# eric-downes/tianshou_marl

Measured on AMD Instinct MI355X. Metric: env-steps/sec (n_env x n_agent) incl. PPO update, simple_spread N=3, higher is better.
Workload: dtype f32; 1 GPU; simple_spread_v3 N=3 shared PPO, num_envs=1024 per GPU, obs 18, A=5, T=25, MLP 64-64; minibatch=4096, repeat=1, dispatch=per_agent, parallelism=env-shard x1

## Files before the change

tianshou_marl_amd/csrc/mlp_tile.h:

```cpp
#pragma once
#include "common.h"

namespace {

typedef float f4 __attribute__((ext_vector_type(4)));

constexpr int R = 16;
constexpr int NT = 256;
constexpr int kMaxJ = 4;

struct Dims {
    int D, A;
    int Kp1;
    int nJ;
    int ld1;
};

__host__ __device__ constexpr Dims dims_const(int D, int A) {
    Dims d{};
    d.D = D; d.A = A; d.Kp1 = (D + 3) / 4 * 4; d.nJ = (D + 15) / 16; d.ld1 = 16 * ((D + 15) / 16) + 2;
    return d;
}

template <int H>
struct Lay {
    static constexpr int ldh = H + 2;
    static constexpr int ld2 = 2 * H + 2;
    static constexpr int ldo = 18;
    int W1, W2a, W2c, W3a, W3c, B1, B2, B3a, B3c, X, H1, H2, OUT, D3, D2, D1, total;
    __host__ __device__ Lay(const Dims &d, bool bwd) {
        int o = 0;
        W1 = o; o += 2 * H * d.ld1;
        W2a = o; o += H * ldh;
        W2c = o; o += H * ldh;
        W3a = o; o += 16 * ldh;
        W3c = o; o += H;
        B1 = o; o += 2 * H;
        B2 = o; o += 2 * H;
        B3a = o; o += 16;
        B3c = o; o += 2;
        o = (o + 3) & ~3;
        X = o; o += R * d.ld1;
        H1 = o; o += R * ld2;
        H2 = o; o += R * ld2;
        OUT = o; o += R * ldo;
        D3 = o; o += bwd ? R * ldo : 0;
        D2 = o; o += bwd ? R * ld2 : 0;
        D1 = o; o += bwd ? R * ld2 : 0;
        total = o;
    }
};

__device__ __forceinline__ f4 mfma(float a, float b, f4 c) {
    return __builtin_amdgcn_mfma_f32_16x16x4f32(a, b, c, 0, 0, 0);
}

template <int N>
__device__ __forceinline__ float fmaf_chain_ahead(const float *h, const float *w) {
    constexpr int Q = 8;
    static_assert(N % (2 * Q) == 0, "pairs of whole groups");
    float h0[Q], w0[Q], h1[Q], w1[Q], s = 0.f;
    int off = 0;
    auto pin = [&]() { asm volatile("" : "+v"(s), "+v"(off)); };
#pragma unroll
    for (int p = 0; p < Q; ++p) { h0[p] = h[p]; w0[p] = w[p]; }
#pragma unroll
    for (int j0 = 0; j0 < N; j0 += 2 * Q) {
        pin();
#pragma unroll
        for (int p = 0; p < Q; ++p) { h1[p] = h[off + j0 + Q + p]; w1[p] = w[off + j0 + Q + p]; }
#pragma unroll
        for (int p = 0; p < Q; ++p) s = fmaf(h0[p], w0[p], s);
        pin();
        if (j0 + 2 * Q < N) {
#pragma unroll
            for (int p = 0; p < Q; ++p) { h0[p] = h[off + j0 + 2 * Q + p]; w0[p] = w[off + j0 + 2 * Q + p]; }
        }
#pragma unroll
        for (int p = 0; p < Q; ++p) s = fmaf(h1[p], w1[p], s);
    }
    return s;
}

template <int H>
struct POff {
    int aW1, ab1, aW2, ab2, aW3, ab3, cW1, cb1, cW2, cb2, cW3, cb3, total;
    __host__ __device__ POff(int D, int A) {
        int o = 0;
        aW1 = o; o += H * D; ab1 = o; o += H; aW2 = o; o += H * H; ab2 = o; o += H; aW3 = o; o += A * H; ab3 = o; o += A;
        cW1 = o; o += H * D; cb1 = o; o += H; cW2 = o; o += H * H; cb2 = o; o += H; cW3 = o; o += H; cb3 = o; o += 1;
        total = o;
    }
};

template <int H>
__device__ void stage_weights(float *lds, const Lay<H> &ly, const Dims &d, const float *__restrict__ P, int tid_in = -1) {
    const POff<H> po(d.D, d.A);
    const int tid = tid_in < 0 ? (int)threadIdx.x : tid_in;
    constexpr int U = 12;
    for (int e0 = tid; e0 < 2 * H * d.ld1; e0 += U * NT) {
        float v[U];
#pragma unroll
        for (int u = 0; u < U; ++u) {
            const int e = e0 + u * NT;
            const int row = e / d.ld1, c = e - row * d.ld1;
            v[u] = 0.f;
            if (e < 2 * H * d.ld1 && c < d.D) v[u] = row < H ? P[po.aW1 + row * d.D + c] : P[po.cW1 + (row - H) * d.D + c];
        }
#pragma unroll
        for (int u = 0; u < U; ++u)
            if (e0 + u * NT < 2 * H * d.ld1) lds[ly.W1 + e0 + u * NT] = v[u];
    }
    for (int e0 = tid; e0 < H * ly.ldh; e0 += U * NT) {
        float va[U], vc[U];
#pragma unroll
        for (int u = 0; u < U; ++u) {
            const int e = e0 + u * NT;
            const int row = e / ly.ldh, c = e - row * ly.ldh;
            const bool on = e < H * ly.ldh && c < H;
            va[u] = on ? P[po.aW2 + row * H + c] : 0.f;
            vc[u] = on ? P[po.cW2 + row * H + c] : 0.f;
        }
#pragma unroll
        for (int u = 0; u < U; ++u) {
            const int e = e0 + u * NT;
            if (e < H * ly.ldh) { lds[ly.W2a + e] = va[u]; lds[ly.W2c + e] = vc[u]; }
        }
    }
    {
        constexpr int N3 = (16 * Lay<H>::ldh + NT - 1) / NT;
        float v3[N3], vv[5];
#pragma unroll
        for (int u = 0; u < N3; ++u) {
            const int e = tid + u * NT, row = e / ly.ldh, c = e - row * ly.ldh;
            v3[u] = (e < 16 * ly.ldh && row < d.A && c < H) ? P[po.aW3 + row * H + c] : 0.f;
        }
        const int e5 = tid < H ? tid : 0;
        vv[0] = P[po.cW3 + e5]; vv[1] = P[po.ab1 + e5]; vv[2] = P[po.cb1 + e5]; vv[3] = P[po.ab2 + e5]; vv[4] = P[po.cb2 + e5];
#pragma unroll
        for (int u = 0; u < N3; ++u) {
            const int e = tid + u * NT;
            if (e < 16 * ly.ldh) lds[ly.W3a + e] = v3[u];
        }
        if (tid < H) {
            lds[ly.W3c + tid] = vv[0]; lds[ly.B1 + tid] = vv[1]; lds[ly.B1 + H + tid] = vv[2]; lds[ly.B2 + tid] = vv[3];
            lds[ly.B2 + H + tid] = vv[4];
        }
    }
    if (tid < 16) lds[ly.B3a + tid] = tid < d.A ? P[po.ab3 + tid] : 0.f;
    if (tid == 0) lds[ly.B3c] = P[po.cb3];
}

constexpr int kStageChunk = 4 * 256;
__host__ __device__ inline int image_f4_padded(int x_floats) {
    return ((x_floats / 4) + kStageChunk - 1) / kStageChunk * kStageChunk;
}

template <int H>
__device__ __forceinline__ void stage_image(float *lds, const Lay<H> &ly, const float *__restrict__ img) {
    const int n4p = image_f4_padded(ly.X);
    const int wave_base = (threadIdx.x >> 6) * 64;
    for (int e = 0; e < n4p; e += NT) {
        __builtin_amdgcn_global_load_lds(
            (const __attribute__((address_space(1))) void *)(img + (size_t)(e + threadIdx.x) * 4),
            (__attribute__((address_space(3))) void *)(lds + (size_t)(e + wave_base) * 4), 16, 0, 0);
    }
}

template <int H>
__device__ __forceinline__ void tile_forward(float *lds, const Lay<H> &ly, const Dims &d) {
    const int lane = threadIdx.x & 63, w = threadIdx.x >> 6;
    const int r16 = lane & 15, kq = lane >> 4;
    {
        f4 acc_a = {0.f, 0.f, 0.f, 0.f}, acc_c = {0.f, 0.f, 0.f, 0.f};
        const float *xa = lds + ly.X + r16 * d.ld1 + kq;
        const float *wa = lds + ly.W1 + (16 * w + r16) * d.ld1 + kq;
        const float *wc = lds + ly.W1 + (H + 16 * w + r16) * d.ld1 + kq;
        for (int k0 = 0; k0 < d.Kp1; k0 += 4) {
            const float a = xa[k0];
            acc_a = mfma(a, wa[k0], acc_a);
            acc_c = mfma(a, wc[k0], acc_c);
        }
        const int col = 16 * w + r16;
        const float ba = lds[ly.B1 + col], bc = lds[ly.B1 + H + col];
#pragma unroll
        for (int r = 0; r < 4; ++r) {
            const int row = kq * 4 + r;
            lds[ly.H1 + row * ly.ld2 + col] = fmaxf(acc_a[r] + ba, 0.f);
            lds[ly.H1 + row * ly.ld2 + H + col] = fmaxf(acc_c[r] + bc, 0.f);
        }
    }
    __syncthreads();
    {
        f4 acc_a = {0.f, 0.f, 0.f, 0.f}, acc_c = {0.f, 0.f, 0.f, 0.f};
        const float *ha = lds + ly.H1 + r16 * ly.ld2 + kq;
        const float *hc = ha + H;
        const float *wa = lds + ly.W2a + (16 * w + r16) * ly.ldh + kq;
        const float *wc = lds + ly.W2c + (16 * w + r16) * ly.ldh + kq;
#pragma unroll
        for (int k0 = 0; k0 < H; k0 += 4) {
            acc_a = mfma(ha[k0], wa[k0], acc_a);
            acc_c = mfma(hc[k0], wc[k0], acc_c);
        }
        const int col = 16 * w + r16;
        const float ba = lds[ly.B2 + col], bc = lds[ly.B2 + H + col];
#pragma unroll
        for (int r = 0; r < 4; ++r) {
            const int row = kq * 4 + r;
            lds[ly.H2 + row * ly.ld2 + col] = fmaxf(acc_a[r] + ba, 0.f);
            lds[ly.H2 + row * ly.ld2 + H + col] = fmaxf(acc_c[r] + bc, 0.f);
        }
    }
    __syncthreads();
    if (w == 0) {
        f4 acc = {0.f, 0.f, 0.f, 0.f};
        const float *ha = lds + ly.H2 + r16 * ly.ld2 + kq;
        const float *wa = lds + ly.W3a + r16 * ly.ldh + kq;
#pragma unroll
        for (int k0 = 0; k0 < H; k0 += 4) acc = mfma(ha[k0], wa[k0], acc);
        const float b = lds[ly.B3a + r16];
#pragma unroll
        for (int r = 0; r < 4; ++r) lds[ly.OUT + (kq * 4 + r) * ly.ldo + r16] = acc[r] + b;
    } else if (w == 1 && lane < R) {
        const float *hc = lds + ly.H2 + lane * ly.ld2 + H;
        float s = 0.f;
        for (int j = 0; j < H; ++j) s = fmaf(hc[j], lds[ly.W3c + j], s);
        lds[ly.OUT + lane * ly.ldo + 16] = s + lds[ly.B3c];
    }
    __syncthreads();
}

template <int H>
__device__ __forceinline__ void tile_forward_split(float *lds, const Lay<H> &ly, const Dims &d) {
    const int lane = threadIdx.x & 63, w8 = threadIdx.x >> 6, net = w8 >> 2, w = w8 & 3;
    const int r16 = lane & 15, kq = lane >> 4;
    const int col = 16 * w + r16;
    {
        f4 acc = {0.f, 0.f, 0.f, 0.f};
        const float *xa = lds + ly.X + r16 * d.ld1 + kq;
        const float *wp = lds + ly.W1 + (net * H + col) * d.ld1 + kq;
        for (int k0 = 0; k0 < d.Kp1; k0 += 4) acc = mfma(xa[k0], wp[k0], acc);
        const float b = lds[ly.B1 + net * H + col];
#pragma unroll
        for (int r = 0; r < 4; ++r) lds[ly.H1 + (kq * 4 + r) * ly.ld2 + net * H + col] = fmaxf(acc[r] + b, 0.f);
    }
    __syncthreads();
    {
        f4 acc = {0.f, 0.f, 0.f, 0.f};
        const float *ha = lds + ly.H1 + r16 * ly.ld2 + net * H + kq;
        const float *wp = lds + (net ? ly.W2c : ly.W2a) + col * ly.ldh + kq;
#pragma unroll
        for (int k0 = 0; k0 < H; k0 += 4) acc = mfma(ha[k0], wp[k0], acc);
        const float b = lds[ly.B2 + net * H + col];
#pragma unroll
        for (int r = 0; r < 4; ++r) lds[ly.H2 + (kq * 4 + r) * ly.ld2 + net * H + col] = fmaxf(acc[r] + b, 0.f);
    }
    __syncthreads();
    if (w8 == 0) {
        f4 acc = {0.f, 0.f, 0.f, 0.f};
        const float *ha = lds + ly.H2 + r16 * ly.ld2 + kq;
        const float *wa = lds + ly.W3a + r16 * ly.ldh + kq;
#pragma unroll
        for (int k0 = 0; k0 < H; k0 += 4) acc = mfma(ha[k0], wa[k0], acc);
        const float b = lds[ly.B3a + r16];
#pragma unroll
        for (int r = 0; r < 4; ++r) lds[ly.OUT + (kq * 4 + r) * ly.ldo + r16] = acc[r] + b;
    } else if (w8 == 5 && lane < R) {
        const float *hc = lds + ly.H2 + lane * ly.ld2 + H;
        float s = 0.f;
        for (int j = 0; j < H; ++j) s = fmaf(hc[j], lds[ly.W3c + j], s);
        lds[ly.OUT + lane * ly.ldo + 16] = s + lds[ly.B3c];
    }
    __syncthreads();
}

constexpr int kXRegs = (R * (16 * kMaxJ + 2) + NT - 1) / NT;

template <int HAS_PERM = -1>
__device__ __forceinline__ void prefetch_tile_ids_load(int64_t (&id)[kXRegs + 1], const Dims &d, const int64_t *__restrict__ perm,
                                                       int64_t first, int64_t row0, int64_t M) {
    const int64_t ir = row0 + (threadIdx.x >> 4);
    if (HAS_PERM == 1 || (HAS_PERM == -1 && perm)) {
#pragma unroll
        for (int it = 0; it < kXRegs; ++it) {
            const int e = threadIdx.x + it * NT, r = e / d.ld1;
            const int64_t i = row0 + r;
            id[it] = perm[(e < R * d.ld1 && i < M) ? i : row0];
        }
        id[kXRegs] = perm[ir < M ? ir : row0];
    } else {
#pragma unroll
        for (int it = 0; it < kXRegs; ++it) id[it] = first + row0 + (threadIdx.x + it * NT) / d.ld1;
        id[kXRegs] = first + ir;
    }
}
__device__ __forceinline__ int64_t prefetch_tile_ids_done(int64_t (&xs)[kXRegs], const int64_t (&id)[kXRegs + 1], const Dims &d,
                                                          int64_t row0, int64_t M) {
#pragma unroll
    for (int it = 0; it < kXRegs; ++it) {
        const int e = threadIdx.x + it * NT, r = e / d.ld1, c = e - r * d.ld1;
        xs[it] = (e < R * d.ld1 && c < d.D && row0 + r < M) ? id[it] * d.D + c : -1;
    }
    return row0 + (threadIdx.x >> 4) < M ? id[kXRegs] : -1;
}
__device__ __forceinline__ int64_t prefetch_tile_ids_done_nb(int64_t (&xs)[kXRegs], unsigned &ok, const int64_t (&id)[kXRegs + 1],
                                                             const Dims &d, int64_t row0, int64_t M) {
    ok = 0;
#pragma unroll
    for (int it = 0; it < kXRegs; ++it) {
        const int e = threadIdx.x + it * NT, r = e / d.ld1, c = e - r * d.ld1;
        xs[it] = id[it] * d.D + (c < d.D ? c : 0);
        ok |= (unsigned)(e < R * d.ld1 && c < d.D && row0 + r < M) << it;
    }
    return row0 + (threadIdx.x >> 4) < M ? id[kXRegs] : -1;
}
__device__ __forceinline__ void prefetch_tile_vals_nb(float (&xr)[kXRegs], const int64_t (&xs)[kXRegs], unsigned ok,
                                                      const float *__restrict__ obs) {
#pragma unroll
    for (int it = 0; it < kXRegs; ++it) {
        const float v = obs[xs[it]];
        xr[it] = (ok >> it & 1u) ? v : 0.f;
    }
}
__device__ __forceinline__ void prefetch_tile_ids(int64_t (&xs)[kXRegs], const Dims &d,
                                                  const int64_t *__restrict__ perm, int64_t first, int64_t row0,
                                                  int64_t M) {
    int64_t id[kXRegs + 1];
    prefetch_tile_ids_load(id, d, perm, first, row0, M);
    (void)prefetch_tile_ids_done(xs, id, d, row0, M);
}

__device__ __forceinline__ void prefetch_tile_vals(float (&xr)[kXRegs], const int64_t (&xs)[kXRegs],
                                                   const float *__restrict__ obs) {
#pragma unroll
    for (int it = 0; it < kXRegs; ++it) {
        const float v = obs[xs[it] >= 0 ? xs[it] : 0];
        xr[it] = xs[it] >= 0 ? v : 0.f;
    }
}

__device__ __forceinline__ void prefetch_tile_x(float (&xr)[kXRegs], const Dims &d, const float *__restrict__ obs,
                                                const int64_t *__restrict__ perm, int64_t first, int64_t row0,
                                                int64_t M) {
    int64_t xs[kXRegs];
    prefetch_tile_ids(xs, d, perm, first, row0, M);
    prefetch_tile_vals(xr, xs, obs);
}

__device__ __forceinline__ void commit_tile_x(float *lds, int X, const Dims &d, const float (&xr)[kXRegs]) {
#pragma unroll
    for (int it = 0; it < kXRegs; ++it) {
        const int e = threadIdx.x + it * NT;
        if (e < R * d.ld1) lds[X + e] = xr[it];
    }
}

__device__ __forceinline__ void load_tile_x(float *lds, int X, const Dims &d, const float *__restrict__ obs,
                                            const int64_t *__restrict__ perm, int64_t first, int64_t row0,
                                            int64_t M) {
    float xr[kXRegs];
    prefetch_tile_x(xr, d, obs, perm, first, row0, M);
    commit_tile_x(lds, X, d, xr);
}

static int make_dims(int32_t obs_dim, int32_t hidden, int32_t n_act, Dims *d) {
    TSM_REQUIRE(hidden == 64, "fused MLP supports hidden == 64 (got %d)", hidden);
    TSM_REQUIRE(obs_dim >= 1 && obs_dim <= 16 * kMaxJ, "fused MLP supports 1 <= obs_dim <= %d (got %d)", 16 * kMaxJ,
                obs_dim);
    TSM_REQUIRE(n_act >= 1 && n_act <= 16, "fused MLP supports 1 <= n_act <= 16 (got %d)", n_act);
    d->D = obs_dim;
    d->A = n_act;
    d->Kp1 = (obs_dim + 3) / 4 * 4;
    d->nJ = (obs_dim + 15) / 16;
    d->ld1 = 16 * d->nJ + 2;
    return TSM_OK;
}


}
```

tianshou_marl_amd/csrc/rollout.hip:

```cpp
#include "common.h"
#include "mlp_tile.h"
#include "mpe_dev.h"
#include "philox.h"
#include "rollout_dev.h"
#include "wave_mlp.h"

int tsm_mpe_check_cfg(const tsm_mpe_cfg *h, MpeCfg *c);
extern long long *g_tsm_stamps;

namespace {

struct RolloutArgs {
    const float *P, *img;
    Dims d;
    uint64_t pol_seed, offset;
    const uint64_t *offset_dev;
    int mode;
    MpeCfg c;
    uint64_t env_seed;
    uint64_t *episode_ctr;
    float *apos, *avel, *lpos;
    int32_t *steps;
    int auto_reset;
    float *obs_cur_out;
    RolloutBufArgs b;
    long long *stamps;
};


#define XSTAMP(k) do { if (a.stamps && blockIdx.x == 0 && threadIdx.x == 0 && t < 4) a.stamps[900 + t * 8 + (k)] = (long long)wall_clock64(); } while (0)
#define STAMP(k) do { if (a.stamps && blockIdx.x == 0 && threadIdx.x == 0 && t < 4) a.stamps[t * 8 + (k)] = (long long)wall_clock64(); } while (0)

struct RtLay {
    int XN0, AP, AV, LP, REW, LOGP, VAL, MIN, ACT, STEPS, DONE, ROW, EP, CX, CY, CV, U, ANY, total;
    __host__ __device__ RtLay(int fwd_total, int ld1) {
        int o = fwd_total;
        XN0 = o; o += R * ld1;
        AP = o; o += R * 2;
        AV = o; o += R * 2;
        LP = o; o += R * 2;
        REW = o; o += R;
        LOGP = o; o += R;
        VAL = o; o += R;
        MIN = o; o += R;
        ACT = o; o += R;
        STEPS = o; o += R;
        DONE = o; o += 2 * R;
        o = (o + 1) & ~1;
        ROW = o; o += 2 * 2 * R;
        EP = o; o += 2 * R;
        o = (o + 3) & ~3;
        CX = o; o += R * 8;
        CY = o; o += R * 8;
        CV = o; o += R * 8;
        U = o; o += 2 * R;
        ANY = o; o += 2;
        o += 3 * R + 12;
        total = o;
    }
};

template <int H, int NT2, int DS = 0, int NS = 0>
__global__ __launch_bounds__(NT2) void rollout_kernel(RolloutArgs a) {
    extern __shared__ __attribute__((aligned(16))) float lds[];
    const Dims d = DS ? dims_const(DS, 5) : a.d;
    MpeCfg c_ = a.c;
    if (NS) { c_.N = NS; c_.obs_dim = DS; }
    const MpeCfg c = c_;
    const Lay<H> ly(d, false);
    const int N = c.N, D = d.D, st = 2 * N;
    const int EPB = R / N;
    const int e0 = blockIdx.x * EPB;
    const int n_here = min(EPB, c.n_env - e0);
    const int rows_here = n_here * N;
    const int64_t B = c.n_env;
    const RtLay tl(ly.total, d.ld1);
    float *XN0 = lds + tl.XN0, *s_ap = lds + tl.AP, *s_av = lds + tl.AV, *s_lp = lds + tl.LP, *s_rew = lds + tl.REW,
          *s_logp = lds + tl.LOGP, *s_val = lds + tl.VAL, *s_m = lds + tl.MIN, *s_cx = lds + tl.CX, *s_cy = lds + tl.CY, *s_u = lds + tl.U;
    int *s_act = reinterpret_cast<int *>(lds + tl.ACT), *s_steps = reinterpret_cast<int *>(lds + tl.STEPS),
        *s_done = reinterpret_cast<int *>(lds + tl.DONE), *s_cv = reinterpret_cast<int *>(lds + tl.CV),
        *s_any = reinterpret_cast<int *>(lds + tl.ANY);
    int64_t *s_row = reinterpret_cast<int64_t *>(lds + tl.ROW);
    uint64_t *s_ep = reinterpret_cast<uint64_t *>(lds + tl.EP);

    if (a.stamps && threadIdx.x == 0 && blockIdx.x < 256) a.stamps[64 + 2 * blockIdx.x] = (long long)wall_clock64();
    const bool main_t = threadIdx.x < NT;
    if (main_t) {
        if (a.img) stage_image<H>(lds, ly, a.img);
        else stage_weights<H>(lds, ly, d, a.P);
    }
    for (int i = threadIdx.x; i < R * d.ld1; i += NT2) { lds[ly.X + i] = 0.f; XN0[i] = 0.f; }
    const VrbState vs = vrb_view(a.b.vrb_state, B, N);
    const int r = threadIdx.x, el = r / N, ai = r - el * N;
    const bool lane_live = r < rows_here;
    const int e = e0 + el;
    constexpr int kEnvBase = NT2 >= 512 ? 256 : 64, kUBase = NT2 >= 512 ? 320 : 128;
    const int bel = (int)threadIdx.x - kEnvBase;
    const bool env_lane = bel >= 0 && bel < n_here;
    const int be = e0 + bel;
    constexpr bool DEFER = NT2 >= 512;
    constexpr int kRewBase = 384;
    const int wl = (int)threadIdx.x - kRewBase;
    const bool rew_lane = DEFER && wl >= 0 && wl < rows_here;
    constexpr int kRetBase = 448;
    const int rl = (int)threadIdx.x - kRetBase;
    const bool ret_lane = DEFER ? (rl >= 0 && rl < n_here) : env_lane;
    const int rq = DEFER ? rl : bel;
    bool pending = false;
    VrbLane vl;
    int n_fin_r = 0;
    EpReturns<kMpeMaxN> epr;
    if (ret_lane) epr.load(vs, N, e0 + rq);
    auto step_returns = [&](int tt, bool trq) {
        const int64_t bq = e0 + rq;
        const bool recq = trq && a.b.ep_rec && n_fin_r < a.b.max_ep;
        epr.fold(a.b.ep_rew_out, a.b.ep_rec, a.b.max_ep, N, B, bq, (int64_t)tt * B + bq, trq, recq, n_fin_r, s_rew + rq * N);
    };
    if (env_lane) {
        vl.load(vs, be);
        s_steps[bel] = a.steps[be];
        s_done[bel] = 1; s_done[R + bel] = 1;
        s_row[bel] = 0; s_row[R + bel] = 0;
    }
    for (int i = threadIdx.x; i < n_here * st; i += NT2) {
        s_ap[i] = a.apos[(int64_t)e0 * st + i];
        s_av[i] = a.avel[(int64_t)e0 * st + i];
        s_lp[i] = a.lpos[(int64_t)e0 * st + i];
    }
    const uint64_t off0 = a.offset + (a.offset_dev ? *a.offset_dev : 0ull);
    const int ur = (int)threadIdx.x - kUBase;
    const bool u_lane = a.mode == 1 && ur >= 0 && ur < rows_here;
    if (u_lane) s_u[ur] = tsm_philox_uniform(a.pol_seed, off0 + (uint64_t)e0 * N + (uint64_t)ur);
    __syncthreads();
    Lay<H> lyf = ly;
    int xcur = ly.X, xnxt = tl.XN0;
    for (int i = threadIdx.x; i < rows_here * D; i += NT2) {
        const int rr = i / D, k = i - rr * D, ee = rr / N;
        lds[xcur + rr * d.ld1 + k] = mpe_obs_elem(c, s_ap + ee * st, s_av + ee * st, s_lp + ee * st, rr - ee * N, k);
    }
    __syncthreads();

    for (int t = 0; t <= a.b.n_steps; ++t) {
        const int g = (t & 1) * R;
        const bool last = t == a.b.n_steps;
        float *XN = lds + xnxt;
        STAMP(0);
        if (a.stamps && blockIdx.x == 0 && threadIdx.x == 0 && t < 64) a.stamps[640 + t] = (long long)wall_clock64();
        STAMP(1);
        lyf.X = xcur;
        if constexpr (NT2 == 2 * NT) tile_forward_split<H>(lds, lyf, d);
        else tile_forward<H>(lds, lyf, d);
        STAMP(2);
        bool tr = false;
        if (env_lane && !last) {
            const int stp = s_steps[bel] + 1;
            tr = stp >= c.max_cycles;
            s_steps[bel] = stp;
            const VrbStep sp = vl.add(vs, a.b.S, t, be, B, tr, a.b.done_store, a.b.ptr_out, a.b.ep_len_out, a.b.ep_idx_out, a.b.ep_rec, a.b.max_ep);
            vl.n_fin += tr ? 1 : 0;
            s_row[g + bel] = sp.row;
            s_done[g + bel] = tr ? 1 : 0;
            const unsigned long long ends = __ballot(tr);
            if (bel == 0) s_any[t & 1] = ends != 0ull;
        }
        if (u_lane && !last) s_u[((t + 1) & 1) * R + ur] = tsm_philox_uniform(a.pol_seed, off0 + (uint64_t)(t + 1) * B * N + (uint64_t)e0 * N + (uint64_t)ur);
        if (DEFER && pending) {
            if (wl >= 0 && wl < 64) {
                const int wr = wl < rows_here ? wl : 0;
                const int wel = wr / N, wai = wr - wel * N;
                const int64_t rowq = s_row[(g ^ R) + wel];
                const MpePos pos = mpe_load_pos(c, s_ap + wel * st);
                const float md = mpe_landmark_min_dist(c, pos, s_lp + wel * st, wai);
                const float local = mpe_local_penalty(c, pos, s_ap + wel * st, wai);
                float mv[kMpeMaxN];
#pragma unroll
                for (int l = 0; l < kMpeMaxN; ++l) mv[l] = l < N ? __shfl(md, wel * N + l, 64) : 0.f;
                const float rw = mpe_reward_regs(c, mv, local);
                if (wl < rows_here) { s_rew[wl] = rw; a.b.rew_store[rowq * N + wai] = rw; }
            }
            pending = false;
        }
        auto pair_task = [&](int p) {
            const int rp = p >> 3, jp = p & 7;
            float sx = 0.f, sy = 0.f;
            int ok = 0;
            if (rp < rows_here && jp < N) {
                const int ep = rp / N, ip = rp - ep * N;
                const float *ap = s_ap + ep * st;
                if (jp != ip) ok = mpe_pair_force(c, ap[2 * ip], ap[2 * ip + 1], ap[2 * jp], ap[2 * jp + 1], ip, jp, sx, sy) ? 1 : 0;
            }
            s_cx[p] = sx; s_cy[p] = sy; s_cv[p] = ok;
        };
        if (DEFER && !last) {
            if (N <= 4) { if (rl >= 0 && rl < 64) pair_task(((rl >> 2) << 3) | (rl & 3)); }
            else if (rl >= 0 && rl < 64) pair_task(rl);
            else if (ur >= 0 && ur < 64) pair_task(64 + ur);
        }
        if (main_t) {
            const int hr = threadIdx.x >> 4, j = threadIdx.x & 15;
            const float *lg = lds + ly.OUT + hr * ly.ldo;
            const bool on = j < d.A;
            const float x = on ? lg[j] : -INFINITY;
            const float m = row16_max(x);
            const float ex = on ? expf(x - m) : 0.f;
            const int gbase = threadIdx.x & 48;
            float ssum = 0.f;
            row_prefix_sum<0>(ex, d.A, ssum);
            if (j == 0 && hr < rows_here) {
                const float val = lg[16];
                const int hel = hr / N;
                if (!s_done[(g ^ R) + hel] && a.b.vnext_store)
                    a.b.vnext_store[s_row[(g ^ R) + hel] * N + (hr - hel * N)] = val;
                if (!last) s_val[hr] = val;
            }
            if (!last) {
                int act = 0;
                if (a.mode == 1) {
                    const float u = s_u[(t & 1) * R + (hr < rows_here ? hr : 0)] * ssum;
                    float cs = 0.f;
                    act = d.A - 1;
                    bool found = false;
                    row_cdf_pick<0>(ex, d.A, u, cs, act, found);
                } else {
                    const unsigned long long eq = __ballot(on && x == m);
                    act = __ffsll((long long)((eq >> gbase) & 0xFFFFull)) - 1;
                }
                const float la = __shfl(x, gbase + act, 64);
                if (j == 0 && hr < rows_here) {
                    s_act[hr] = act;
                    s_logp[hr] = la - (m + logf(ssum));
                }
            }
        }
        __syncthreads();
        STAMP(3);
        if (DEFER && t > 0 && ret_lane) {
            step_returns(t - 1, s_done[(g ^ R) + rq] != 0);
        }
        if (last) {
            if (a.obs_cur_out)
                for (int i = threadIdx.x; i < rows_here * D; i += NT2) {
                    const int rr = i / D, k = i - rr * D;
                    a.obs_cur_out[((int64_t)e0 * N + rr) * D + k] = lds[xcur + rr * d.ld1 + k];
                }
            break;
        }
        if constexpr (!DEFER) {
            if (threadIdx.x < R * 8) pair_task(threadIdx.x);
            XSTAMP(5);
            __syncthreads();
        }
        XSTAMP(0);
        if (lane_live) {
            const float px = s_ap[el * st + 2 * ai], py = s_ap[el * st + 2 * ai + 1];
            const float vx = s_av[el * st + 2 * ai], vy = s_av[el * st + 2 * ai + 1];
            float fx = mpe_action_force(c, s_act[r], 0);
            float fy = mpe_action_force(c, s_act[r], 1);
            mpe_pair_fold(c, s_cx, s_cy, s_cv, r, fx, fy);
            float npx, npy, nvx, nvy;
            mpe_integrate(c, px, py, vx, vy, fx, fy, npx, npy, nvx, nvy);
            s_ap[el * st + 2 * ai] = npx; s_ap[el * st + 2 * ai + 1] = npy;
            s_av[el * st + 2 * ai] = nvx; s_av[el * st + 2 * ai + 1] = nvy;
        }
        __syncthreads();
        XSTAMP(1);
        const int any_done = s_any[t & 1];
        const bool now = !DEFER || any_done;
        if (now) {
            float local = 0.f;
            if (lane_live) {
                const MpePos pos = mpe_load_pos(c, s_ap + el * st);
                s_m[r] = mpe_landmark_min_dist(c, pos, s_lp + el * st, ai);
                local = mpe_local_penalty(c, pos, s_ap + el * st, ai);
            }
            XSTAMP(2);
            if (!DEFER && threadIdx.x >= 64)
                for (int i = threadIdx.x - 64; i < rows_here * D; i += NT2 - 64) {
                    const int rr = i / D, k = i - rr * D, ee = rr / N;
                    XN[rr * d.ld1 + k] =
                        mpe_obs_elem(c, s_ap + ee * st, s_av + ee * st, s_lp + ee * st, rr - ee * N, k);
                }
            __syncthreads();
            XSTAMP(3);
            if (lane_live) s_rew[r] = mpe_reward(c, s_m + el * N, local);
            __syncthreads();
            XSTAMP(4);
            if (!DEFER && ret_lane) {
                step_returns(t, s_done[g + rq] != 0);
            }
        }
        STAMP(4);
        for (int i = threadIdx.x; i < rows_here * D; i += NT2) {
            const int rr = i / D, k = i - rr * D, ee = rr / N;
            float v;
            if constexpr (DEFER) {
                v = mpe_obs_elem(c, s_ap + ee * st, s_av + ee * st, s_lp + ee * st, rr - ee * N, k);
                XN[rr * d.ld1 + k] = v;
            } else {
                v = XN[rr * d.ld1 + k];
            }
            const int64_t dst = (s_row[g + ee] * N + (rr - ee * N)) * D + k;
            a.b.obs_store[dst] = lds[xcur + rr * d.ld1 + k];
            if (a.b.obs_next_store) a.b.obs_next_store[dst] = v;
        }
        if (ur >= 0 && ur < rows_here) {
            const int pel = ur / N, pai = ur - pel * N;
            const int64_t dst = s_row[g + pel] * N + pai;
            a.b.act_store[dst] = s_act[ur];
            if (now) a.b.rew_store[dst] = s_rew[ur];
            a.b.term_store[dst] = 0;
            a.b.trunc_store[dst] = (uint8_t)s_done[g + pel];
            if (a.b.logp_store) a.b.logp_store[dst] = s_logp[ur];
            if (a.b.vs_store) a.b.vs_store[dst] = s_val[ur];
        }
        if constexpr (DEFER) __syncthreads();
        pending = !now;
        STAMP(5);
        if (any_done) {
            if (a.b.vnext_store) {
                lyf.X = xnxt;
                if constexpr (NT2 == 2 * NT) tile_forward_split<H>(lds, lyf, d);
                else tile_forward<H>(lds, lyf, d);
                if (lane_live && s_done[g + el]) a.b.vnext_store[s_row[g + el] * N + ai] = lds[ly.OUT + r * ly.ldo + 16];
            }
            if (a.auto_reset) {
                if (env_lane && s_done[g + bel]) {
                    const uint64_t ep = a.episode_ctr[be];
                    s_ep[bel] = ep;
                    a.episode_ctr[be] = ep + 1;
                    s_steps[bel] = 0;
                }
                __syncthreads();
                if (lane_live && s_done[g + el])
                    mpe_reset_agent(c, e, a.env_seed, s_ep[el], ai, s_ap + el * st, s_av + el * st, s_lp + el * st);
                __syncthreads();
                for (int i = threadIdx.x; i < rows_here * D; i += NT2) {
                    const int rr = i / D, k = i - rr * D, ee = rr / N;
                    if (s_done[g + ee])
                        XN[rr * d.ld1 + k] =
                            mpe_obs_elem(c, s_ap + ee * st, s_av + ee * st, s_lp + ee * st, rr - ee * N, k);
                }
                __syncthreads();
            }
        }
        { const int tmp = xcur; xcur = xnxt; xnxt = tmp; }
        STAMP(6);
    }
    __syncthreads();
    if (a.stamps && threadIdx.x == 0 && blockIdx.x < 256) a.stamps[65 + 2 * blockIdx.x] = (long long)wall_clock64();
    for (int i = threadIdx.x; i < n_here * st; i += NT2) {
        a.apos[(int64_t)e0 * st + i] = s_ap[i];
        a.avel[(int64_t)e0 * st + i] = s_av[i];
        a.lpos[(int64_t)e0 * st + i] = s_lp[i];
    }
    if (env_lane) {
        a.steps[be] = s_steps[bel];
        vl.store(vs, a.b.ep_rec, be);
    }
    if (ret_lane) epr.store(vs, N, e0 + rq);
    rollout_advance_counter(a.b.done_ctr, a.b.offset_dev_rw, a.b.offset_inc, threadIdx.x == 0);
}

struct Rw64Lay {
    static constexpr int kLdc = 68;
    int AP, AV, LP, LG, H2C, VAL, CX, CY, CV, MIN, REW, LOGP, ACT, STEPS, DONE, ROW, EP, size;
    __host__ __device__ Rw64Lay() {
        int q = 0;
        AP = q; q += 2 * R;
        AV = q; q += 2 * R;
        LP = q; q += 2 * R;
        LG = q; q += R * 16;
        H2C = q; q += R * kLdc;
        VAL = q; q += R;
        CX = q; q += R * 8;
        CY = q; q += R * 8;
        CV = q; q += R * 8;
        MIN = q; q += R;
        REW = q; q += R;
        LOGP = q; q += R;
        ACT = q; q += R;
        STEPS = q; q += R;
        DONE = q; q += R;
        ROW = q; q += 2 * R;
        EP = q; q += 2 * R;
        size = (q + 3) & ~3;
    }
};

template <int NJ, int DS = 0, int NS = 0>
__global__ __launch_bounds__(NT) void rollout_wave64_kernel(RolloutArgs a) {
    constexpr int H = 64, MB = H / 16, KB1 = 4 * NJ, KBH = H / 4;
    extern __shared__ __attribute__((aligned(16))) float lds[];
    const Dims d = DS ? dims_const(DS, 5) : a.d;
    MpeCfg c_ = a.c;
    if (NS) { c_.N = NS; c_.obs_dim = DS; }
    const MpeCfg c = c_;
    const Lay<H> ly(d, false);
    const Rw64Lay wl;
    constexpr int ld1 = 16 * NJ + 2;
    const int tid = threadIdx.x, lane = tid & 63, w = tid >> 6, n_waves = blockDim.x >> 6, c16 = lane & 15, kq = lane >> 4;
    const int N = c.N, D = d.D, A = d.A, st = 2 * N;
    const int EPW = R / N;
    const int e0 = (blockIdx.x * n_waves + w) * EPW;
    const int n_here = max(0, min(EPW, c.n_env - e0));
    const int rows_here = n_here * N;
    const int64_t B = c.n_env;
    const int img_floats = image_f4_padded(ly.X) * 4;
    if (a.img) {
        const int n4p = img_floats / 4, wave_base = w * 64;
        for (int e = 0; e < n4p; e += blockDim.x)
            __builtin_amdgcn_global_load_lds((const __attribute__((address_space(1))) void *)(a.img + (size_t)(e + tid) * 4),
                                             (__attribute__((address_space(3))) void *)(lds + (size_t)(e + wave_base) * 4), 16, 0, 0);
    } else {
        for (int v = tid; v < NT; v += blockDim.x) stage_weights<H>(lds, ly, d, a.P, v);
    }
    const int wvo = img_floats + w * wl.size;
    float *wv = lds + wvo;
    float *s_ap = wv + wl.AP, *s_av = wv + wl.AV, *s_lp = wv + wl.LP, *s_lg = wv + wl.LG, *s_h2c = wv + wl.H2C, *s_val = wv + wl.VAL,
          *s_cx = wv + wl.CX, *s_cy = wv + wl.CY, *s_m = wv + wl.MIN, *s_rew = wv + wl.REW, *s_logp = wv + wl.LOGP;
    int *s_cv = reinterpret_cast<int *>(wv + wl.CV), *s_act = reinterpret_cast<int *>(wv + wl.ACT),
        *s_steps = reinterpret_cast<int *>(wv + wl.STEPS), *s_done = reinterpret_cast<int *>(wv + wl.DONE);
    int64_t *s_row = reinterpret_cast<int64_t *>(wv + wl.ROW);
    uint64_t *s_ep = reinterpret_cast<uint64_t *>(wv + wl.EP);

    const VrbState vs = vrb_view(a.b.vrb_state, B, N);
    const int r = lane, el = r / N, ai = r - el * N;
    const bool lane_live = r < rows_here;
    const int e = e0 + el;
    const int bel = lane - 16;
    const bool env_lane = bel >= 0 && bel < n_here;
    const int be = e0 + bel;
    VrbLane vl;
    EpReturns<kMpeMaxN> epr;
    if (env_lane) {
        vl.load(vs, be);
        epr.load(vs, N, be);
    }
    float st_ap = 0.f, st_av = 0.f, st_lp = 0.f;
    if (lane < n_here * st) {
        st_ap = a.apos[(int64_t)e0 * st + lane]; st_av = a.avel[(int64_t)e0 * st + lane]; st_lp = a.lpos[(int64_t)e0 * st + lane];
    }
    const int steps0 = env_lane ? a.steps[be] : 0;
    const uint64_t off0 = a.offset + (a.offset_dev ? *a.offset_dev : 0ull);
    __syncthreads();
    if (n_here == 0) return;
    if (env_lane) { s_steps[bel] = steps0; s_done[bel] = 1; s_row[bel] = 0; }
    if (lane < n_here * st) { s_ap[lane] = st_ap; s_av[lane] = st_av; s_lp[lane] = st_lp; }
    if (lane < 16) s_lg[16 * 16 - 1 - lane] = 0.f;

    const int zoff = wvo + wl.LG + 16 * 15 + 15;
    uint32_t el_ab[KB1];
    const int sn_el = c16 / N, sn_ai = c16 - sn_el * N;
    const bool sn_live = c16 < rows_here;
#pragma unroll
    for (int kb = 0; kb < KB1; ++kb) {
        const int k = 4 * kb + kq;
        const int base = wvo + sn_el * st;
        el_ab[kb] = sn_live && k < D ? mpe_obs_offsets(N, base + wl.AP, base + wl.AV, base + wl.LP, zoff, sn_ai, k) : mpe_obs_offsets_zero(zoff);
    }
    const int ND = N * D;
    const int obs_col = sn_ai * D + kq;
    int pair_ei[2];
#pragma unroll
    for (int q = 0; q < 2; ++q) {
        const int rp = (lane + 64 * q) >> 3, ep = rp / N;
        pair_ei[q] = rp < rows_here ? (ep << 3) | (rp - ep * N) : -1;
    }
    const int kb1_n = d.Kp1 >> 2;
    const float *w1a = lds + ly.W1 + c16 * ld1 + kq, *w1c = w1a + H * ld1;
    const float *w2a = lds + ly.W2a + c16 * ly.ldh + kq, *w2c = lds + ly.W2c + c16 * ly.ldh + kq, *w3a = lds + ly.W3a + c16 * ly.ldh + kq;
    auto critic_value = [&](const float (&x)[KB1]) -> float {
        wf4 acc[MB];
        float hb[4 * MB];
        wave_layer<MB, KB1>(w1c, ld1, x, kb1_n, acc);
        wave_bias_relu<MB, true>(lds + ly.B1 + H + 4 * kq, acc);
        wave_to_frags<MB>(acc, hb);
        wave_layer<MB, KBH>(w2c, ly.ldh, hb, KBH, acc);
        wave_bias_relu<MB, true>(lds + ly.B2 + H + 4 * kq, acc);
#pragma unroll
        for (int mb = 0; mb < MB; ++mb) *reinterpret_cast<wf4 *>(s_h2c + c16 * Rw64Lay::kLdc + 16 * mb + 4 * kq) = acc[mb];
        float s = 0.f;
        if (lane < R) {
            wf4 hv[H / 4], wq[H / 4];
#pragma unroll
            for (int q = 0; q < H / 4; ++q) {
                hv[q] = *reinterpret_cast<const wf4 *>(s_h2c + lane * Rw64Lay::kLdc + 4 * q);
                wq[q] = *reinterpret_cast<const wf4 *>(lds + ly.W3c + 4 * q);
            }
#pragma unroll
            for (int j = 0; j < H; ++j) s = fmaf(hv[j >> 2][j & 3], wq[j >> 2][j & 3], s);
            s += lds[ly.B3c];
        }
        return s;
    };

    for (int t = 0; t <= a.b.n_steps; ++t) {
        const bool last = t == a.b.n_steps;
        int64_t p_row = 0;
        int p_done = 1;
        if (lane_live) { p_row = s_row[el]; p_done = s_done[el]; }
        bool tr = false, rec = false;
        int64_t o = 0;
        if (env_lane && !last) {
            const int stp = s_steps[bel] + 1;
            tr = stp >= c.max_cycles;
            s_steps[bel] = stp;
            const VrbStep sp = vl.add(vs, a.b.S, t, be, B, tr, a.b.done_store, a.b.ptr_out, a.b.ep_len_out, a.b.ep_idx_out, a.b.ep_rec, a.b.max_ep);
            o = sp.o; rec = sp.rec;
            s_row[bel] = sp.row;
            s_done[bel] = tr ? 1 : 0;
        }
        float xb[KB1];
        wave_obs_frags(lds, el_ab, xb);
        if (last) {
            if (a.obs_cur_out && sn_live) wave_obs_rows_out(a.obs_cur_out + ((int64_t)e0 * N + c16) * D + kq, xb, D, kq);
        } else if (sn_live) {
            wave_obs_rows_out(a.b.obs_store + s_row[sn_el] * ND + obs_col, xb, D, kq);
        }
        const float val = critic_value(xb);
        if (lane_live && !p_done && a.b.vnext_store) a.b.vnext_store[p_row * N + ai] = val;
        if (last) break;
        {
            wf4 acc[MB];
            float hb[4 * MB];
            wave_layer<MB, KB1>(w1a, ld1, xb, kb1_n, acc);
            wave_bias_relu<MB, true>(lds + ly.B1 + 4 * kq, acc);
            wave_to_frags<MB>(acc, hb);
            wave_layer<MB, KBH>(w2a, ly.ldh, hb, KBH, acc);
            wave_bias_relu<MB, true>(lds + ly.B2 + 4 * kq, acc);
            wave_to_frags<MB>(acc, hb);
            wf4 lg = wf4{0.f, 0.f, 0.f, 0.f};
#pragma unroll
            for (int kb = 0; kb < KBH; ++kb) lg = wave_mfma4(w3a[4 * kb], hb[kb], lg);
            const wf4 b = *reinterpret_cast<const wf4 *>(lds + ly.B3a + 4 * kq);
            if (!(c16 == 15 && kq == 3))
                *reinterpret_cast<wf4 *>(s_lg + c16 * 16 + 4 * kq) = wf4{lg[0] + b[0], lg[1] + b[1], lg[2] + b[2], lg[3] + b[3]};
        }
        if (lane_live) {
            float lgv[8], ex[8];
            {
                const wf4 l0 = *reinterpret_cast<const wf4 *>(s_lg + lane * 16), l1 = *reinterpret_cast<const wf4 *>(s_lg + lane * 16 + 4);
                lgv[0] = l0[0]; lgv[1] = l0[1]; lgv[2] = l0[2]; lgv[3] = l0[3]; lgv[4] = l1[0]; lgv[5] = l1[1]; lgv[6] = l1[2]; lgv[7] = l1[3];
            }
            float m = -INFINITY;
            int arg = 0;
#pragma unroll
            for (int j = 0; j < 8; ++j) if (j < A && lgv[j] > m) { m = lgv[j]; arg = j; }
            float s = 0.f;
#pragma unroll
            for (int j = 0; j < 8; ++j) { ex[j] = 0.f; if (j < A) { ex[j] = expf(lgv[j] - m); s += ex[j]; } }
            const float lse = m + logf(s);
            int act = arg;
            if (a.mode == 1) {
                const uint64_t gi = (uint64_t)e0 * N + (uint64_t)lane;
                const float u = tsm_philox_uniform(a.pol_seed, off0 + (uint64_t)t * B * N + gi) * s;
                float cs = 0.f;
                bool found = false;
                act = A - 1;
#pragma unroll
                for (int j = 0; j < 8; ++j)
                    if (j < A) {
                        cs += ex[j];
                        if (!found && u < cs) { act = j; found = true; }
                    }
            }
            float la = lgv[0];
#pragma unroll
            for (int j = 1; j < 8; ++j) la = act == j ? lgv[j] : la;
            s_act[lane] = act;
            s_logp[lane] = la - lse;
            s_val[lane] = val;
        }
        mpe_pair_tasks(c, pair_ei, lane, 64, s_ap, s_cx, s_cy, s_cv);
        if (lane_live) {
            const float px = s_ap[el * st + 2 * ai], py = s_ap[el * st + 2 * ai + 1];
            const float vx = s_av[el * st + 2 * ai], vy = s_av[el * st + 2 * ai + 1];
            float fx = mpe_action_force(c, s_act[r], 0);
            float fy = mpe_action_force(c, s_act[r], 1);
            mpe_pair_fold(c, s_cx, s_cy, s_cv, r, fx, fy);
            float npx, npy, nvx, nvy;
            mpe_integrate(c, px, py, vx, vy, fx, fy, npx, npy, nvx, nvy);
            s_ap[el * st + 2 * ai] = npx; s_ap[el * st + 2 * ai + 1] = npy;
            s_av[el * st + 2 * ai] = nvx; s_av[el * st + 2 * ai + 1] = nvy;
        }
        float local = 0.f;
        if (lane_live) {
            const MpePos pos = mpe_load_pos(c, s_ap + el * st);
            s_m[r] = mpe_landmark_min_dist(c, pos, s_lp + el * st, ai);
            local = mpe_local_penalty(c, pos, s_ap + el * st, ai);
        }
        float xn[KB1];
        const unsigned long long done_mask = __ballot(lane_live && s_done[el]);
        if (a.b.obs_next_store || (done_mask && a.b.vnext_store)) wave_obs_frags(lds, el_ab, xn);
        if (a.b.obs_next_store && sn_live) wave_obs_rows_out(a.b.obs_next_store + s_row[sn_el] * ND + obs_col, xn, D, kq);
        if (lane_live) {
            float mv[kMpeMaxN];
#pragma unroll
            for (int l = 0; l < kMpeMaxN; ++l) mv[l] = s_m[el * N + (l < N ? l : N - 1)];
            float global = 0.f;
#pragma unroll
            for (int l = 0; l < kMpeMaxN; ++l) if (l < N) global -= mv[l];
            s_rew[r] = global * (1.f - c.local_ratio) + local * c.local_ratio;
        }
        if (env_lane) epr.fold(a.b.ep_rew_out, a.b.ep_rec, a.b.max_ep, N, B, be, o, tr, rec, vl.n_fin, s_rew + bel * N);
        if (lane_live) {
            const int64_t dst = s_row[el] * N + ai;
            a.b.act_store[dst] = s_act[r];
            a.b.rew_store[dst] = s_rew[r];
            a.b.term_store[dst] = 0;
            a.b.trunc_store[dst] = (uint8_t)s_done[el];
            if (a.b.logp_store) a.b.logp_store[dst] = s_logp[r];
            if (a.b.vs_store) a.b.vs_store[dst] = s_val[r];
        }
        if (done_mask) {
            if (a.b.vnext_store) {
                const float vt = critic_value(xn);
                if (lane_live && s_done[el]) a.b.vnext_store[s_row[el] * N + ai] = vt;
            }
            if (a.auto_reset) {
                if (env_lane && s_done[bel]) {
                    const uint64_t ep = a.episode_ctr[be];
                    s_ep[bel] = ep;
                    a.episode_ctr[be] = ep + 1;
                    s_steps[bel] = 0;
                }
                if (lane_live && s_done[el])
                    mpe_reset_agent(c, e, a.env_seed, s_ep[el], ai, s_ap + el * st, s_av + el * st, s_lp + el * st);
            }
        }
    }
    if (lane < n_here * st) {
        a.apos[(int64_t)e0 * st + lane] = s_ap[lane];
        a.avel[(int64_t)e0 * st + lane] = s_av[lane];
        a.lpos[(int64_t)e0 * st + lane] = s_lp[lane];
    }
    if (env_lane) {
        a.steps[be] = s_steps[bel];
        vl.store(vs, a.b.ep_rec, be);
        epr.store(vs, N, be);
    }
    rollout_advance_counter(a.b.done_ctr, a.b.offset_dev_rw, a.b.offset_inc, tid == 0);
}

__global__ void u64_add_kernel(uint64_t *p, uint64_t inc) { *p += inc; }

}

TSM_EXPORT int tsm_u64_add(uint64_t *counter, uint64_t inc, void *stream) {
    TSM_REQUIRE(counter, "tsm_u64_add: null pointer");
    hipLaunchKernelGGL(u64_add_kernel, dim3(1), dim3(1), 0, tsm_stream(stream), counter, inc);
    TSM_LAUNCH_CHECK();
    return TSM_OK;
}

TSM_EXPORT int tsm_rollout_spread(const tsm_rollout_desc *desc_host, void *stream) {
    TSM_REQUIRE(desc_host, "tsm_rollout_spread: null descriptor");
    const tsm_rollout_desc &h = *desc_host;
    RolloutArgs a;
    if (int rc = make_dims(h.obs_dim, h.hidden, h.n_act, &a.d)) return rc;
    if (int rc = tsm_mpe_check_cfg(&h.env, &a.c)) return rc;
    TSM_REQUIRE(a.c.obs_dim == h.obs_dim, "tsm_rollout_spread: obs_dim %d != 6 * n_agent", h.obs_dim);
    TSM_REQUIRE(h.n_act == 5, "tsm_rollout_spread: simple_spread has 5 discrete actions");
    TSM_REQUIRE(a.c.N <= R, "tsm_rollout_spread: n_agent exceeds the row tile");
    TSM_REQUIRE(h.n_steps >= 1 && h.sub_size >= 1, "tsm_rollout_spread: bad n_steps / sub_size");
    TSM_REQUIRE(h.mode == 1 || h.mode == 2, "tsm_rollout_spread: mode must be 1 (sample) or 2 (argmax)");
    TSM_REQUIRE((h.params || h.param_image) && h.episode_ctr && h.agent_pos && h.agent_vel && h.landmark_pos && h.steps,
                "tsm_rollout_spread: null pointer");
    if (int rc = rollout_buf_args(h, "tsm_rollout_spread", &a.b)) return rc;
    a.P = h.params; a.img = h.param_image;
    a.pol_seed = h.policy_seed; a.offset = h.offset; a.offset_dev = h.offset_dev; a.mode = h.mode;
    a.env_seed = h.env_seed; a.episode_ctr = h.episode_ctr;
    a.apos = h.agent_pos; a.avel = h.agent_vel; a.lpos = h.landmark_pos; a.steps = h.steps;
    a.auto_reset = h.auto_reset; a.obs_cur_out = h.obs_cur_out;
    a.stamps = g_tsm_stamps;
    const Lay<64> ly(a.d, false);
    {
        const int form = tsm_opt(TSM_OPT_ROLLOUT_FORM);
        const int64_t total_waves = ceil_div(a.c.n_env, R / a.c.N);
        if (a.d.nJ <= 3 && (form == 2 || (form == 0 && total_waves > 256))) {
            int n_waves = 1;
            while (n_waves < 4 && ceil_div(total_waves, n_waves) > 256) n_waves *= 2;
            const Rw64Lay wl;
            const size_t shmem_w = ((size_t)image_f4_padded(ly.X) * 4 + (size_t)n_waves * wl.size) * sizeof(float);
            TSM_REQUIRE(shmem_w <= kTsmMaxLds, "tsm_rollout_spread: LDS layout of %zu bytes does not fit", shmem_w);
            const unsigned n_wg_w = (unsigned)ceil_div(total_waves, n_waves);
            static bool attr_w[4] = {false, false, false, false};
#define LAUNCHW(NJ)                                                                                                    \
    do {                                                                                                               \
        if (!attr_w[NJ - 1]) {                                                                                         \
            TSM_HIP(tsm_allow_max_lds(reinterpret_cast<const void *>(rollout_wave64_kernel<NJ>)));                    \
            attr_w[NJ - 1] = true;                                                                                     \
        }                                                                                                              \
        hipLaunchKernelGGL((rollout_wave64_kernel<NJ>), dim3(n_wg_w), dim3(64 * n_waves), shmem_w, tsm_stream(stream), a); \
    } while (0)
            if (a.d.D == 18 && a.d.A == 5 && a.c.N == 3 && !tsm_opt(TSM_OPT_GENERIC)) {
                static bool attr_18 = false;
                if (!attr_18) {
                    TSM_HIP(tsm_allow_max_lds(reinterpret_cast<const void *>(rollout_wave64_kernel<2, 18, 3>)));
                    attr_18 = true;
                }
                hipLaunchKernelGGL((rollout_wave64_kernel<2, 18, 3>), dim3(n_wg_w), dim3(64 * n_waves), shmem_w, tsm_stream(stream), a);
            } else
            switch (a.d.nJ) {
                case 1: LAUNCHW(1); break;
                case 2: LAUNCHW(2); break;
                default: LAUNCHW(3); break;
            }
#undef LAUNCHW
            TSM_LAUNCH_CHECK();
            return TSM_OK;
        }
    }
    const size_t shmem = (size_t)RtLay(ly.total, a.d.ld1).total * sizeof(float);
    static bool attr_set = false;
    if (!attr_set) {
        TSM_HIP(tsm_allow_max_lds(reinterpret_cast<const void *>(rollout_kernel<64, NT>)));
        TSM_HIP(tsm_allow_max_lds(reinterpret_cast<const void *>(rollout_kernel<64, 2 * NT>)));
        TSM_HIP(tsm_allow_max_lds(reinterpret_cast<const void *>(rollout_kernel<64, 2 * NT, 18, 3>)));
        attr_set = true;
    }
    const int EPB = R / a.c.N;
    const unsigned n_wg = (unsigned)ceil_div(a.c.n_env, EPB);
    const bool eight = n_wg <= 256 || shmem > 80 * 1024;
    const bool c18 = a.d.D == 18 && a.d.A == 5 && a.c.N == 3 && !tsm_opt(TSM_OPT_GENERIC);
    if (eight && c18) hipLaunchKernelGGL((rollout_kernel<64, 2 * NT, 18, 3>), dim3(n_wg), dim3(2 * NT), shmem, tsm_stream(stream), a);
    else if (eight) hipLaunchKernelGGL((rollout_kernel<64, 2 * NT>), dim3(n_wg), dim3(2 * NT), shmem, tsm_stream(stream), a);
    else hipLaunchKernelGGL((rollout_kernel<64, NT>), dim3(n_wg), dim3(NT), shmem, tsm_stream(stream), a);
    TSM_LAUNCH_CHECK();
    return TSM_OK;
}
```

Measured before the change: 162.6 million env-steps/s.

## Split actor and critic forward so critic overlaps sampling and env step

Splits the fused actor+critic tile forward into separate actor and critic phases in the deferred rollout path. Only the actor runs on the critical path before action sampling. The critic's layers run on the non-main warps while sampling and returns are computed, and the value head is evaluated later, with vs and vnext stores moved accordingly. This aims to shorten the per-step serial chain at the cost of more complex synchronisation and a risk of LDS races between the critic writes and other phases.

New measurement: 156.7 million env-steps/s. -3.7%, worse.

```diff
diff --git a/tianshou_marl_amd/csrc/mlp_tile.h b/tianshou_marl_amd/csrc/mlp_tile.h
--- a/tianshou_marl_amd/csrc/mlp_tile.h
+++ b/tianshou_marl_amd/csrc/mlp_tile.h
@@ -231,47 +231,85 @@
 }
 
 template <int H>
+__device__ __forceinline__ void tile_split_l1(float *lds, const Lay<H> &ly, const Dims &d, int net, int w) {
+    const int lane = threadIdx.x & 63, r16 = lane & 15, kq = lane >> 4;
+    const int col = 16 * w + r16;
+    f4 acc = {0.f, 0.f, 0.f, 0.f};
+    const float *xa = lds + ly.X + r16 * d.ld1 + kq;
+    const float *wp = lds + ly.W1 + (net * H + col) * d.ld1 + kq;
+    for (int k0 = 0; k0 < d.Kp1; k0 += 4) acc = mfma(xa[k0], wp[k0], acc);
+    const float b = lds[ly.B1 + net * H + col];
+#pragma unroll
+    for (int r = 0; r < 4; ++r) lds[ly.H1 + (kq * 4 + r) * ly.ld2 + net * H + col] = fmaxf(acc[r] + b, 0.f);
+}
+template <int H>
+__device__ __forceinline__ void tile_split_l2(float *lds, const Lay<H> &ly, int net, int w) {
+    const int lane = threadIdx.x & 63, r16 = lane & 15, kq = lane >> 4;
+    const int col = 16 * w + r16;
+    f4 acc = {0.f, 0.f, 0.f, 0.f};
+    const float *ha = lds + ly.H1 + r16 * ly.ld2 + net * H + kq;
+    const float *wp = lds + (net ? ly.W2c : ly.W2a) + col * ly.ldh + kq;
+#pragma unroll
+    for (int k0 = 0; k0 < H; k0 += 4) acc = mfma(ha[k0], wp[k0], acc);
+    const float b = lds[ly.B2 + net * H + col];
+#pragma unroll
+    for (int r = 0; r < 4; ++r) lds[ly.H2 + (kq * 4 + r) * ly.ld2 + net * H + col] = fmaxf(acc[r] + b, 0.f);
+}
+template <int H>
+__device__ __forceinline__ void tile_split_logits(float *lds, const Lay<H> &ly) {
+    const int lane = threadIdx.x & 63, r16 = lane & 15, kq = lane >> 4;
+    f4 acc = {0.f, 0.f, 0.f, 0.f};
+    const float *ha = lds + ly.H2 + r16 * ly.ld2 + kq;
+    const float *wa = lds + ly.W3a + r16 * ly.ldh + kq;
+#pragma unroll
+    for (int k0 = 0; k0 < H; k0 += 4) acc = mfma(ha[k0], wa[k0], acc);
+    const float b = lds[ly.B3a + r16];
+#pragma unroll
+    for (int r = 0; r < 4; ++r) lds[ly.OUT + (kq * 4 + r) * ly.ldo + r16] = acc[r] + b;
+}
+template <int H>
+__device__ __forceinline__ float tile_split_value(float *lds, const Lay<H> &ly, int row) {
+    const float *hc = lds + ly.H2 + row * ly.ld2 + H;
+    float s = 0.f;
+    for (int j = 0; j < H; ++j) s = fmaf(hc[j], lds[ly.W3c + j], s);
+    s += lds[ly.B3c];
+    lds[ly.OUT + row * ly.ldo + 16] = s;
+    return s;
+}
+
+template <int H>
 __device__ __forceinline__ void tile_forward_split(float *lds, const Lay<H> &ly, const Dims &d) {
     const int lane = threadIdx.x & 63, w8 = threadIdx.x >> 6, net = w8 >> 2, w = w8 & 3;
-    const int r16 = lane & 15, kq = lane >> 4;
-    const int col = 16 * w + r16;
-    {
-        f4 acc = {0.f, 0.f, 0.f, 0.f};
-        const float *xa = lds + ly.X + r16 * d.ld1 + kq;
-        const float *wp = lds + ly.W1 + (net * H + col) * d.ld1 + kq;
-        for (int k0 = 0; k0 < d.Kp1; k0 += 4) acc = mfma(xa[k0], wp[k0], acc);
-        const float b = lds[ly.B1 + net * H + col];
-#pragma unroll
-        for (int r = 0; r < 4; ++r) lds[ly.H1 + (kq * 4 + r) * ly.ld2 + net * H + col] = fmaxf(acc[r] + b, 0.f);
-    }
-    __syncthreads();
-    {
-        f4 acc = {0.f, 0.f, 0.f, 0.f};
-        const float *ha = lds + ly.H1 + r16 * ly.ld2 + net * H + kq;
-        const float *wp = lds + (net ? ly.W2c : ly.W2a) + col * ly.ldh + kq;
-#pragma unroll
-        for (int k0 = 0; k0 < H; k0 += 4) acc = mfma(ha[k0], wp[k0], acc);
-        const float b = lds[ly.B2 + net * H + col];
-#pragma unroll
-        for (int r = 0; r < 4; ++r) lds[ly.H2 + (kq * 4 + r) * ly.ld2 + net * H + col] = fmaxf(acc[r] + b, 0.f);
-    }
-    __syncthreads();
-    if (w8 == 0) {
-        f4 acc = {0.f, 0.f, 0.f, 0.f};
-        const float *ha = lds + ly.H2 + r16 * ly.ld2 + kq;
-        const float *wa = lds + ly.W3a + r16 * ly.ldh + kq;
-#pragma unroll
-        for (int k0 = 0; k0 < H; k0 += 4) acc = mfma(ha[k0], wa[k0], acc);
-        const float b = lds[ly.B3a + r16];
-#pragma unroll
-        for (int r = 0; r < 4; ++r) lds[ly.OUT + (kq * 4 + r) * ly.ldo + r16] = acc[r] + b;
-    } else if (w8 == 5 && lane < R) {
-        const float *hc = lds + ly.H2 + lane * ly.ld2 + H;
-        float s = 0.f;
-        for (int j = 0; j < H; ++j) s = fmaf(hc[j], lds[ly.W3c + j], s);
-        lds[ly.OUT + lane * ly.ldo + 16] = s + lds[ly.B3c];
-    }
-    __syncthreads();
+    tile_split_l1<H>(lds, ly, d, net, w);
+    __syncthreads();
+    tile_split_l2<H>(lds, ly, net, w);
+    __syncthreads();
+    if (w8 == 0) tile_split_logits<H>(lds, ly);
+    else if (w8 == 5 && lane < R) {
+        (void)tile_split_value<H>(lds, ly, lane);
+    }
+    __syncthreads();
+}
+
+template <int H>
+__device__ __forceinline__ void tile_forward_actor(float *lds, const Lay<H> &ly, const Dims &d) {
+    const int w8 = threadIdx.x >> 6;
+    if (w8 < 4) tile_split_l1<H>(lds, ly, d, 0, w8);
+    __syncthreads();
+    if (w8 < 4) tile_split_l2<H>(lds, ly, 0, w8);
+    __syncthreads();
+    if (w8 == 0) tile_split_logits<H>(lds, ly);
+    __syncthreads();
+}
+
+template <int H>
+__device__ __forceinline__ float tile_forward_critic(float *lds, const Lay<H> &ly, const Dims &d) {
+    const int lane = threadIdx.x & 63, w8 = threadIdx.x >> 6;
+    if (w8 >= 4) tile_split_l1<H>(lds, ly, d, 1, w8 & 3);
+    __syncthreads();
+    if (w8 >= 4) tile_split_l2<H>(lds, ly, 1, w8 & 3);
+    __syncthreads();
+    return (w8 == 5 && lane < R) ? tile_split_value<H>(lds, ly, lane) : 0.f;
 }
 
 constexpr int kXRegs = (R * (16 * kMaxJ + 2) + NT - 1) / NT;
diff --git a/tianshou_marl_amd/csrc/rollout.hip b/tianshou_marl_amd/csrc/rollout.hip
--- a/tianshou_marl_amd/csrc/rollout.hip
+++ b/tianshou_marl_amd/csrc/rollout.hip
@@ -148,7 +148,7 @@
         if (a.stamps && blockIdx.x == 0 && threadIdx.x == 0 && t < 64) a.stamps[640 + t] = (long long)wall_clock64();
         STAMP(1);
         lyf.X = xcur;
-        if constexpr (NT2 == 2 * NT) tile_forward_split<H>(lds, lyf, d);
+        if constexpr (DEFER) { if (!last) tile_forward_actor<H>(lds, lyf, d); }
         else tile_forward<H>(lds, lyf, d);
         STAMP(2);
         bool tr = false;
@@ -196,7 +196,18 @@
             else if (rl >= 0 && rl < 64) pair_task(rl);
             else if (ur >= 0 && ur < 64) pair_task(64 + ur);
         }
-        if (main_t) {
+        auto value_stores = [&](float val, bool cur) {
+            if (ur >= 0 && ur < rows_here) {
+                const int pel = ur / N, pai = ur - pel * N;
+                if (!s_done[(g ^ R) + pel] && a.b.vnext_store) a.b.vnext_store[s_row[(g ^ R) + pel] * N + pai] = val;
+                if (cur && a.b.vs_store) a.b.vs_store[s_row[g + pel] * N + pai] = val;
+            }
+        };
+        if constexpr (DEFER) {
+            if (last) value_stores(tile_forward_critic<H>(lds, lyf, d), false);
+            else if (!main_t) tile_split_l1<H>(lds, lyf, d, 1, (threadIdx.x >> 6) & 3);
+        }
+        if (main_t && !(DEFER && last)) {
             const int hr = threadIdx.x >> 4, j = threadIdx.x & 15;
             const float *lg = lds + ly.OUT + hr * ly.ldo;
             const bool on = j < d.A;
@@ -206,7 +217,7 @@
             const int gbase = threadIdx.x & 48;
             float ssum = 0.f;
             row_prefix_sum<0>(ex, d.A, ssum);
-            if (j == 0 && hr < rows_here) {
+            if (!DEFER && j == 0 && hr < rows_here) {
                 const float val = lg[16];
                 const int hel = hr / N;
                 if (!s_done[(g ^ R) + hel] && a.b.vnext_store)
@@ -237,6 +248,7 @@
         if (DEFER && t > 0 && ret_lane) {
             step_returns(t - 1, s_done[(g ^ R) + rq] != 0);
         }
+        if (DEFER && !last && !main_t) tile_split_l2<H>(lds, lyf, 1, (threadIdx.x >> 6) & 3);
         if (last) {
             if (a.obs_cur_out)
                 for (int i = threadIdx.x; i < rows_here * D; i += NT2) {
@@ -311,17 +323,24 @@
             a.b.term_store[dst] = 0;
             a.b.trunc_store[dst] = (uint8_t)s_done[g + pel];
             if (a.b.logp_store) a.b.logp_store[dst] = s_logp[ur];
-            if (a.b.vs_store) a.b.vs_store[dst] = s_val[ur];
-        }
-        if constexpr (DEFER) __syncthreads();
+            if (!DEFER && a.b.vs_store) a.b.vs_store[dst] = s_val[ur];
+        }
+        if constexpr (DEFER) {
+            if (ur >= 0 && ur < R) value_stores(tile_split_value<H>(lds, lyf, ur), true);
+            __syncthreads();
+        }
         pending = !now;
         STAMP(5);
         if (any_done) {
             if (a.b.vnext_store) {
                 lyf.X = xnxt;
-                if constexpr (NT2 == 2 * NT) tile_forward_split<H>(lds, lyf, d);
-                else tile_forward<H>(lds, lyf, d);
-                if (lane_live && s_done[g + el]) a.b.vnext_store[s_row[g + el] * N + ai] = lds[ly.OUT + r * ly.ldo + 16];
+                if constexpr (DEFER) {
+                    const float vt = tile_forward_critic<H>(lds, lyf, d);
+                    if (ur >= 0 && ur < rows_here && s_done[g + ur / N]) a.b.vnext_store[s_row[g + ur / N] * N + (ur - ur / N * N)] = vt;
+                } else {
+                    tile_forward<H>(lds, lyf, d);
+                    if (lane_live && s_done[g + el]) a.b.vnext_store[s_row[g + el] * N + ai] = lds[ly.OUT + r * ly.ldo + 16];
+                }
             }
             if (a.auto_reset) {
                 if (env_lane && s_done[g + bel]) {
```
